# daigo0927/pwcnet

Hardware: AMD Instinct MI355X
Metric: image_pairs_per_sec_448x1024 (higher is better)
Workload: dtype f32 via fp16x2-split MFMA (fp32 tensors and accumulation; big stride-1 convs, level-1 extractor and correlation on the F16 pipe)

## Files before the change

### include/pwc_hip.h

```cpp
#ifndef PWC_HIP_H
#define PWC_HIP_H

#include <stddef.h>
#include <stdint.h>

#ifdef __cplusplus
extern "C" {
#endif

typedef void* pwc_stream_t;

enum {
    PWC_OK = 0,
    PWC_EINVAL = -1,
    PWC_EALIGN = -2,
    PWC_ERANGE = -3,
    PWC_EUNSUPPORTED = -4
};

int pwc_version(void);
const char* pwc_error_string(int code);

int pwc_cost_volume_f32(const float* f0, int f0_cs, const float* f1w, int f1w_cs,
                        float* out, int out_cs, int N, int H, int W, int C,
// ... 86 lines not shown
size_t pwc_conv3x3_h2_workspace_floats(int N, int H, int W, int Cin_phys, int Cout, int dilation);
int pwc_conv3x3_h2_supported(int N, int H, int W, int Cin_phys, int Cout, int dilation);
#define PWC_STATUS_NONFINITE 1u
#define PWC_STATUS_STREAMK_TIMEOUT 2u
int pwc_conv3x3_h2_ex_f32(const float* x, int x_cs, int Cin_a_phys, const float* x2, int x2_cs,
                          const float* packed_w, const float* bias, float* y, int y_cs, int N, int H, int W,
                          int Cin_phys, int Cout, int dilation, int apply_act, float slope, float* workspace,
                          size_t workspace_floats, uint32_t* status, pwc_stream_t stream);
int pwc_conv3x3_h2_ex3_f32(const float* x, int x_cs, int Cin_a_phys, const float* x2, int x2_cs, int Cin_b_phys,
                           const float* x3, int x3_cs, const float* packed_w, const float* bias, float* y, int y_cs,
                           int N, int H, int W, int Cin_phys, int Cout, int apply_act, float slope, float* workspace,
                           size_t workspace_floats, uint32_t* status, pwc_stream_t stream);
size_t pwc_conv3x3_c16pair_packed_floats(void);
int pwc_conv3x3_c16pair_pack_f32(const float* w1_hwio, const float* w2_hwio, float* packed, pwc_stream_t stream);
int pwc_conv3x3_c16pair_f32(const float* x, int x_cs, const float* packed, const float* bias1, const float* bias2,
                            float* y, int y_cs, int N, int H, int W, float slope, pwc_stream_t stream);
int pwc_conv3x3_c16pair_supported(int N, int H, int W);
size_t pwc_conv3x3_c3c16pair_packed_floats(void);
int pwc_conv3x3_c3c16pair_pack_f32(const float* w0_hwio, const float* w1_hwio, const float* w2_hwio, float* packed,
                                   pwc_stream_t stream);
int pwc_conv3x3_c3c16pair_f32(const float* x_a, int N_a, const float* x_b, int N_b, const float* packed,
                              const float* bias0, const float* bias1, const float* bias2, float* y, int y_cs,
                              int H0, int W0, float slope, pwc_stream_t stream);
int pwc_conv3x3_c3c16pair_supported(int N, int H0, int W0);
size_t pwc_conv3x3_h2_stride2_packed_floats(int Cin_phys, int Cout);
int pwc_conv3x3_h2_stride2_pack_f32(const float* w_hwio, const int32_t* cin_map, int Cin, int Cin_phys,
                                    int Cout, float* packed_w, pwc_stream_t stream);
size_t pwc_conv3x3_h2_stride2_workspace_floats(int N, int H, int W, int Cin_phys, int Cout);
int pwc_conv3x3_h2_stride2_f32(const float* x, int x_cs, const float* packed_w, const float* bias,
                               float* y, int y_cs, int N, int H, int W, int Cin_phys, int Cout,
                               int apply_act, float slope, float* workspace, size_t workspace_floats,
                               uint32_t* status, pwc_stream_t stream);
int pwc_conv3x3_h2_stride2_supported(int N, int H, int W, int Cin_phys, int Cout);

size_t pwc_conv3x3_sk_packed_floats(int Cin_phys, int Cout);
int pwc_conv3x3_sk_pack_f32(const float* w_hwio, const int32_t* cin_map, int Cin, int Cin_phys, int Cout,
                            float* packed_w, pwc_stream_t stream);
int pwc_conv3x3_sk_f32(const float* x, int x_cs, const float* packed_w, const float* bias, float* y, int y_cs,
                       int N, int H, int W, int Cin_phys, int Cout, int stride, int dilation, int apply_act,
                       float slope, pwc_stream_t stream);
int pwc_conv3x3_sk_supported(int N, int H, int W, int Cin_phys, int Cout, int stride, int dilation);
int pwc_conv3x3_sk_variant_f32(const float* x, int x_cs, const float* packed_w, const float* bias, float* y, int y_cs,
                               int N, int H, int W, int Cin_phys, int Cout, int stride, int dilation, int apply_act,
                               float slope, int tile, pwc_stream_t stream);

size_t pwc_conv3x3_t32_packed_floats(int Cin_phys);
int pwc_conv3x3_t32_pack_f32(const float* w_hwio, const int32_t* cin_map, int Cin, int Cin_phys, float* packed_w,
                             pwc_stream_t stream);
int pwc_conv3x3_t32_f32(const float* x, int x_cs, const float* packed_w, const float* bias, float* y, int y_cs,
                        int N, int H, int W, int Cin_phys, int Cout, int stride, int apply_act, float slope,
                        pwc_stream_t stream);
int pwc_conv3x3_t32_supported(int N, int H, int W, int Cin_phys, int Cout, int stride);
size_t pwc_conv3x3_w32_packed_floats(int Cin_phys);
int pwc_conv3x3_w32_pack_f32(const float* w_hwio, const int32_t* cin_map, int Cin, int Cin_phys, float* packed_w,
                             pwc_stream_t stream);
int pwc_conv3x3_w32_f32(const float* x, int x_cs, const float* packed_w, const float* bias, float* y, int y_cs,
                        int N, int H, int W, int Cin_phys, int Cout, int apply_act, float slope, pwc_stream_t stream);
int pwc_conv3x3_w32_supported(int N, int H, int W, int Cin_phys, int Cout, int stride, int dilation);
int pwc_conv3x3_h2_plan(int N, int H, int W, int Cin_phys, int Cout, int dilation);
int pwc_conv3x3_h2_variant_f32(const float* x, int x_cs, const float* packed_w, const float* bias,
                               float* y, int y_cs, int N, int H, int W, int Cin_phys, int Cout,
                               int dilation, int apply_act, float slope, int variant, float* workspace,
                               size_t workspace_floats, pwc_stream_t stream);
int pwc_conv3x3_wino_split_plan(int N, int H, int W, int Cin_phys, int Cout, int dilation);
size_t pwc_conv3x3_wino_split_workspace_floats(int N, int H, int W, int Cout, int csplit);
int pwc_conv3x3_wino_split_f32(const float* x, int x_cs, const float* packed_u, const float* bias,
// ... 176 lines not shown
```

### pwcnet_amd/_lib.py

```python
import ctypes
import os
import subprocess

import torch

_HERE = os.path.dirname(os.path.abspath(__file__))
CSRC = os.path.join(_HERE, "csrc")
HARNESS = os.environ.get("PWC_HARNESS", "") == "1"
LIB_PATH = os.path.join(CSRC, "libpwc_hip_harness.so" if HARNESS else "libpwc_hip.so")
HARNESS_SIGNATURES_NAMES = ("pwc_debug_cost_volume_blk_rows", "pwc_debug_conv3x3_sk_tile", "pwc_debug_conv3x3_t32",
                            "pwc_debug_h2_reserve_cus", "pwc_debug_conv3x3_s2_tile")
SOURCES = ["conv3x3_mfma.hip", "conv3x3_wino.hip", "conv3x3_direct.hip", "cost_volume.hip", "pwc_ops.hip",
           "pwc_backward.hip", "conv3x3_wgrad.hip", "conv3x3_h2.hip", "conv3x3_c16pair.hip", "conv3x3_sk.hip", "conv3x3_s2.hip", "conv3x3_t32.hip", "conv3x3_w32.hip",
           "pwc_flow_loss.hip", "pwc_unsup.hip", "pwc_census.hip", "pwc_ssim.hip", "pwc_fbcheck.hip", "pwc_fit.hip", "pwc_augment.hip", "pwc_splat.hip", "pwc_pyramid.hip"]
HEADERS = ["pwc_common.h", "conv_fp32_common.h", "cost_volume_common.h", "loss_common.h", "cost_volume_roll.hip", "cost_volume_mfma.hip", "cost_volume_h2.hip", "cost_volume_blk.hip", "conv3x3_wino4.hip", os.path.join("..", "..", "include", "pwc_hip.h")]

_vp, _i, _f, _l, _sz = ctypes.c_void_p, ctypes.c_int, ctypes.c_float, ctypes.c_long, ctypes.c_size_t

SIGNATURES = {
    "pwc_version": (_i, []),
    "pwc_error_string": (ctypes.c_char_p, [_i]),
    "pwc_cost_volume_f32": (_i, [_vp, _i, _vp, _i, _vp, _i, _i, _i, _i, _i, _i, _f, _vp]),
    "pwc_cost_volume_uses_rolling_kernel": (_i, [_i, _i, _i, _i, _i, _i, _i]),
    "pwc_warp_bilinear_f32": (_i, [_vp, _i, _vp, _i, _f, _vp, _i, _i, _i, _i, _i, _vp]),
    "pwc_warp_nearest_f32": (_i, [_vp, _i, _vp, _i, _f, _vp, _i, _i, _i, _i, _i, _vp]),
    "pwc_cost_volume_coarse_f32": (_i, [_vp, _i, _vp, _i, _vp, _i, _f, _vp, _i, _vp, _i, _i, _i, _i, _i, _i, _f, _vp]),
    "pwc_resize_bilinear_pair_f32": (_i, [_vp, _i, _vp, _i, _vp, _i, _vp, _i, _i, _i, _i, _i, _i, _i, _vp]),
    "pwc_warp_copy_f32": (_i, [_i, _vp, _i, _vp, _i, _f, _vp, _i, _i, _i, _i, _i, _vp, _i, _vp, _i, _i, _vp]),
    "pwc_warp_cost_volume_f32": (_i, [_vp, _i, _vp, _i, _vp, _i, _f, _vp, _i, _i, _i, _i, _i, _i, _f, _vp]),
    "pwc_warp_cost_volume_concat_f32": (_i, [_vp, _i, _vp, _i, _vp, _i, _f, _vp, _i, _i, _vp, _i, _i, _i, _i, _i, _i, _f, _vp]),
    "pwc_warp_cost_volume_concat_h2_f32": (_i, [_vp, _i, _vp, _i, _vp, _i, _f, _vp, _i, _i, _vp, _i, _i, _i, _i, _i, _i, _f, _vp]),
    "pwc_warp_cost_volume_concat_blk_f32": (_i, [_vp, _i, _vp, _i, _vp, _i, _f, _vp, _i, _i, _vp, _i, _i, _i, _i, _i, _i, _f, _vp]),
    "pwc_warp_cost_volume_concat_supported": (_i, [_i, _i, _i, _i, _i, _i, _i, _i, _i]),
    "pwc_warp_cost_volume_concat_blk_supported": (_i, [_i, _i, _i, _i, _i, _i, _i, _i, _i]),
    "pwc_conv3x3_packed_floats": (_sz, [_i, _i]),
    "pwc_conv3x3_pack_f32": (_i, [_vp, _vp, _i, _i, _i, _vp, _vp]),
    "pwc_conv3x3_f32": (_i, [_vp, _i, _vp, _vp, _vp, _i, _i, _i, _i, _i, _i, _i, _i, _i, _f, _i, _i, _vp, _sz, _vp]),
    "pwc_conv3x3_workspace_floats": (_sz, [_i, _i]),
    "pwc_conv3x3_plan": (_i, [_i, _i, _i, ctypes.POINTER(_i)]),
    "pwc_conv3x3_uses_halo_kernel": (_i, [_i, _i, _i, _i, _i]),
    "pwc_conv3x3_tile_shape": (_i, [_i, ctypes.POINTER(_i), ctypes.POINTER(_i)]),
    "pwc_conv3x3_wino_packed_floats": (_sz, [_i, _i]),
    "pwc_conv3x3_wino_pack_f32": (_i, [_vp, _vp, _i, _i, _i, _vp, _vp]),
    "pwc_conv3x3_wino_f32": (_i, [_vp, _i, _vp, _vp, _vp, _i, _i, _i, _i, _i, _i, _i, _i, _f, _vp]),
    "pwc_conv3x3_wino_workgroups": (_l, [_i, _i, _i, _i, _i]),
    "pwc_conv3x3_wino4_packed_floats": (_sz, [_i, _i]),
    "pwc_conv3x3_wino4_pack_f32": (_i, [_vp, _vp, _i, _i, _i, _vp, _vp]),
    "pwc_conv3x3_wino4_f32": (_i, [_vp, _i, _vp, _vp, _vp, _i, _i, _i, _i, _i, _i, _i, _i, _f, _vp]),
    "pwc_conv3x3_wino4_supported": (_i, [_i, _i, _i, _i, _i, _i]),
    "pwc_conv3x3_h2_packed_floats": (_sz, [_i, _i]),
    "pwc_conv3x3_h2_pack_f32": (_i, [_vp, _vp, _i, _i, _i, _vp, _vp]),
    "pwc_conv3x3_h2_f32": (_i, [_vp, _i, _vp, _vp, _vp, _i, _i, _i, _i, _i, _i, _i, _i, _f, _vp, _sz, _vp]),
    "pwc_conv3x3_h2_ex_f32": (_i, [_vp, _i, _i, _vp, _i, _vp, _vp, _vp, _i, _i, _i, _i, _i, _i, _i, _i, _f, _vp, _sz, _vp, _vp]),
    "pwc_conv3x3_h2_ex3_f32": (_i, [_vp, _i, _i, _vp, _i, _i, _vp, _i, _vp, _vp, _vp, _i, _i, _i, _i, _i, _i, _i, _f, _vp, _sz, _vp, _vp]),
    "pwc_conv3x3_h2_workspace_floats": (_sz, [_i, _i, _i, _i, _i, _i]),
    "pwc_conv3x3_h2_supported": (_i, [_i, _i, _i, _i, _i, _i]),
    "pwc_conv3x3_h2_plan": (_i, [_i, _i, _i, _i, _i, _i]),
    "pwc_conv3x3_h2_stride2_f32": (_i, [_vp, _i, _vp, _vp, _vp, _i, _i, _i, _i, _i, _i, _i, _f, _vp, _sz, _vp, _vp]),
    "pwc_conv3x3_h2_stride2_supported": (_i, [_i, _i, _i, _i, _i]),
    "pwc_conv3x3_sk_packed_floats": (_sz, [_i, _i]),
    "pwc_conv3x3_sk_pack_f32": (_i, [_vp, _vp, _i, _i, _i, _vp, _vp]),
    "pwc_conv3x3_sk_f32": (_i, [_vp, _i, _vp, _vp, _vp, _i, _i, _i, _i, _i, _i, _i, _i, _i, _f, _vp]),
    "pwc_conv3x3_sk_supported": (_i, [_i, _i, _i, _i, _i, _i, _i]),
    "pwc_conv3x3_sk_variant_f32": (_i, [_vp, _i, _vp, _vp, _vp, _i, _i, _i, _i, _i, _i, _i, _i, _i, _f, _i, _vp]),
    "pwc_conv3x3_t32_packed_floats": (_sz, [_i]),
    "pwc_conv3x3_t32_pack_f32": (_i, [_vp, _vp, _i, _i, _vp, _vp]),
    "pwc_conv3x3_t32_f32": (_i, [_vp, _i, _vp, _vp, _vp, _i, _i, _i, _i, _i, _i, _i, _i, _f, _vp]),
    "pwc_conv3x3_t32_supported": (_i, [_i, _i, _i, _i, _i, _i]),
    "pwc_conv3x3_w32_packed_floats": (_sz, [_i]),
    "pwc_conv3x3_w32_pack_f32": (_i, [_vp, _vp, _i, _i, _vp, _vp]),
    "pwc_conv3x3_w32_f32": (_i, [_vp, _i, _vp, _vp, _vp, _i, _i, _i, _i, _i, _i, _i, _f, _vp]),
    "pwc_conv3x3_w32_supported": (_i, [_i, _i, _i, _i, _i, _i, _i]),
    "pwc_conv3x3_h2_stride2_packed_floats": (_sz, [_i, _i]),
    "pwc_conv3x3_h2_stride2_pack_f32": (_i, [_vp, _vp, _i, _i, _i, _vp, _vp]),
    "pwc_conv3x3_h2_stride2_workspace_floats": (_sz, [_i, _i, _i, _i, _i]),
    "pwc_conv3x3_c16pair_packed_floats": (_sz, []),
    "pwc_conv3x3_c16pair_pack_f32": (_i, [_vp, _vp, _vp, _vp]),
    "pwc_conv3x3_c16pair_f32": (_i, [_vp, _i, _vp, _vp, _vp, _vp, _i, _i, _i, _i, _f, _vp]),
    "pwc_conv3x3_c16pair_supported": (_i, [_i, _i, _i]),
    "pwc_conv3x3_c3c16pair_packed_floats": (_sz, []),
    "pwc_conv3x3_c3c16pair_pack_f32": (_i, [_vp, _vp, _vp, _vp, _vp]),
    "pwc_conv3x3_c3c16pair_f32": (_i, [_vp, _i, _vp, _i, _vp, _vp, _vp, _vp, _vp, _i, _i, _i, _f, _vp]),
    "pwc_conv3x3_c3c16pair_supported": (_i, [_i, _i, _i]),
    "pwc_conv3x3_h2_variant_f32": (_i, [_vp, _i, _vp, _vp, _vp, _i, _i, _i, _i, _i, _i, _i, _i, _f, _i, _vp, _sz, _vp]),
    "pwc_conv3x3_wino_split_plan": (_i, [_i, _i, _i, _i, _i, _i]),
    "pwc_conv3x3_wino_split_workspace_floats": (_sz, [_i, _i, _i, _i, _i]),
    "pwc_conv3x3_wino_split_f32": (_i, [_vp, _i, _vp, _vp, _vp, _i, _i, _i, _i, _i, _i, _i, _i, _f, _i, _vp, _sz, _vp]),
    "pwc_conv3x3_direct_f32": (_i, [_vp, _i, _vp, _vp, _vp, _i, _vp, _i, _i, _i, _i, _i, _i, _i, _i, _i, _f, _vp]),
    "pwc_resize_bilinear_f32": (_i, [_vp, _i, _vp, _i, _i, _i, _i, _i, _i, _i, _f, _vp]),
    "pwc_resize_bilinear_status_f32": (_i, [_vp, _i, _vp, _i, _i, _i, _i, _i, _i, _i, _f, _vp, _vp]),
    "pwc_absmax_f32": (_i, [_vp, _i, _l, _i, _vp, _vp]),
    "pwc_copy_channels_f32": (_i, [_vp, _i, _vp, _i, _l, _i, _vp]),
# ... 140 lines not shown
```

### pwcnet_amd/csrc/conv3x3_h2.hip

```cpp
#pragma once
#include "pwc_common.h"
#include <type_traits>

typedef float pwc_f32x16 __attribute__((ext_vector_type(16)));

struct H2Args {
    const float* x;
    const void* wp;
    const float* bias;
    float* y;
    int x_cs, y_cs;
    int N, H, W;
    int Cin_phys, Cout;
    int apply_act;
    float slope;
    int tiles_x, tiles_y, ncb;
    int dil_y, dil_x;
    int ntiles;
    float* ws_partial;
    unsigned* dbg;
    int Ho, Wo;
    const float* x2;
    int x2_cs, nc16_a;
    const float* x3;
// ... 590 lines not shown
static unsigned* h2_debug_counters = nullptr;
#else
constexpr unsigned* h2_debug_counters = nullptr;
#endif

template <int CT, int PT, int WCG, int ABL, int XS = 1, bool S2 = false>
static int h2_launch(H2Args& a, int hs, int ws, float* workspace, size_t workspace_floats, hipStream_t stream) {
    typedef H2Cfg<CT, PT, WCG, XS> C;
    a.tiles_x = (ws + 31) / 32; a.tiles_y = (hs + C::TR - 1) / C::TR; a.ncb = a.Cout / (32 * C::NCT);
    const long nblk = (long)a.N * a.dil_y * a.dil_x * a.tiles_x * a.tiles_y * a.ncb;
    if (nblk * (a.Cin_phys >> 4) >= (1L << 31)) return PWC_ERANGE;
    a.ntiles = (int)nblk;
    const int cus = h2_cu_count();
    int grid = a.ntiles;
    a.ws_partial = nullptr;
    const size_t part = (size_t)C::NCT * 32 * C::TR * 32;
    if (workspace && h2_split_pays(a.ntiles, a.Cin_phys >> 4, cus) && workspace_floats >= (size_t)cus * part) {
        grid = cus;
        a.ws_partial = workspace;
    }
    pwc_allow_dynamic_lds<&conv3x3_h2_kernel<CT, PT, WCG, ABL, XS, S2>>(C::LDS);
    hipLaunchKernelGGL((conv3x3_h2_kernel<CT, PT, WCG, ABL, XS, S2>), dim3((unsigned)grid), dim3(512), C::LDS, stream, a);
    return pwc_launch_status();
}

static bool h2s2_tile_routed(int N, int H, int W, int x_cs, int Cin_phys, int Cout) {
    const bool ok = h2s2_has_tile_image(Cin_phys, Cout) && pwc_conv3x3_s2_tile_admits(N, H, W, x_cs, Cin_phys, Cout);
#ifdef PWC_HARNESS
    if (pwc_conv3x3_s2_tile_debug_mode()) return ok && pwc_conv3x3_s2_tile_debug_mode() > 0;
#endif
    return ok && Cin_phys == 32;
}

template <int ABL = 0>
static int h2_run(const float* x, int x_cs, const float* packed_w, const float* bias, float* y, int y_cs, int N, int H, int W,
                  int Cin_phys, int Cout, int dilation, int apply_act, float slope, pwc_stream_t stream, int variant = 0,
                  float* workspace = nullptr, size_t workspace_floats = 0, int stride = 1, const float* x2 = nullptr, int x2_cs = 0,
                  int Cin_a_phys = 0, uint32_t* status = nullptr, const float* x3 = nullptr, int x3_cs = 0, int Cin_b_phys = 0) {
    if (!x || !packed_w || !bias || !y) return PWC_EINVAL;
    if (x3 && !x2) return PWC_EINVAL;
    const int slack = x3 ? 12 : 0;
    if (x2) {
        const int cb = x3 ? Cin_b_phys : Cin_phys - Cin_a_phys;
        if (Cin_a_phys <= 0 || Cin_a_phys >= Cin_phys || (Cin_a_phys % 16) || x_cs < Cin_a_phys - slack || x2_cs < cb - slack) return PWC_EINVAL;
        if ((x2_cs & 3) || !pwc_aligned16(x2)) return PWC_EALIGN;
        if ((long)H * W * x2_cs * 4 >= (long)PWC_OOB) return PWC_ERANGE;
    }
    if (x3) {
        const int cc = Cin_phys - Cin_a_phys - Cin_b_phys;
        if (Cin_b_phys <= 0 || (Cin_b_phys % 16) || cc <= 0 || x3_cs < cc - 12 || dilation != 1) return PWC_EINVAL;
        if ((x3_cs & 3) || !pwc_aligned16(x3)) return PWC_EALIGN;
        if ((long)H * W * x3_cs * 4 >= (long)PWC_OOB) return PWC_ERANGE;
    }
    if (reinterpret_cast<uintptr_t>(status) & 7u) return PWC_EALIGN;
    if (dilation < 1 || (stride != 1 && stride != 2)) return PWC_EINVAL;
    const bool shape_ok = !(Cin_phys % 16 || Cout % 32 || Cout > H2_MAX_COUT || (stride == 2 && (dilation != 1 || (H & 1) || (W & 1) || x2)));
    if (const int rc = pwc_conv_io_check(x, x_cs, x2 ? Cin_a_phys - slack : Cin_phys, y, y_cs, Cout, packed_w, bias, N, H, W, shape_ok)) return rc;
    if (!pwc_aligned16(workspace)) return PWC_EALIGN;
    if (((long)H * W + W + 2) * x_cs * 4 >= (long)PWC_OOB || (long)H * W * y_cs * 4 >= (long)PWC_OOB) return PWC_ERANGE;
    H2Args a;
    a.x = x; a.wp = packed_w; a.bias = bias; a.y = y; a.x_cs = x_cs; a.y_cs = y_cs;
    a.N = N; a.H = H; a.W = W; a.Cin_phys = Cin_phys; a.Cout = Cout; a.apply_act = apply_act; a.slope = slope;
    const bool s2 = stride == 2;
    a.Ho = s2 ? H / 2 : H; a.Wo = s2 ? W / 2 : W;
    if (s2) a.Cin_phys = 4 * Cin_phys;
    const H2Geo geo = h2_geometry(a.Ho, a.Wo, dilation, Cout);
    a.dil_y = geo.dy; a.dil_x = geo.dx;
    a.dbg = h2_debug_counters;
    a.x2 = x2; a.x2_cs = x2_cs; a.nc16_a = x2 ? Cin_a_phys >> 4 : a.Cin_phys >> 4; a.status = status;
    a.x3 = x3; a.x3_cs = x3_cs; a.nc16_b = x3 ? Cin_b_phys >> 4 : (a.Cin_phys >> 4) - a.nc16_a;
    const int hs = geo.hs, ws = geo.ws;
    if (variant == 0) variant = h2_plan(N, a.Ho, a.Wo, a.Cin_phys, Cout, dilation, nullptr);
    if (variant < 1 || variant > 5) return PWC_EUNSUPPORTED;
    if (Cout % h2_variant(variant).couts) return PWC_EUNSUPPORTED;
    if (s2 && h2s2_tile_routed(N, H, W, x_cs, Cin_phys, Cout))
        return pwc_conv3x3_s2_tile_launch(x, x_cs, packed_w + h2s2_tile_image_offset(Cin_phys, Cout), bias, y, y_cs, N, H, W, Cin_phys,
                                          Cout, apply_act, slope, stream);
    if (s2) {
        switch (variant) {
            case 1: return h2_launch<2, 2, 2, ABL, 1, true>(a, hs, ws, workspace, workspace_floats, (hipStream_t)stream);
            case 2: return h2_launch<2, 2, 1, ABL, 1, true>(a, hs, ws, workspace, workspace_floats, (hipStream_t)stream);
            case 3: return h2_launch<3, 1, 1, ABL, 1, true>(a, hs, ws, workspace, workspace_floats, (hipStream_t)stream);
            case 4: return h2_launch<1, 2, 1, ABL, 1, true>(a, hs, ws, workspace, workspace_floats, (hipStream_t)stream);
            default: return h2_launch<1, 2, 2, ABL, 1, true>(a, hs, ws, workspace, workspace_floats, (hipStream_t)stream);
        }
    }
    if (geo.xs == 2) {
        switch (variant) {
            case 1: return h2_launch<2, 2, 2, ABL, 2>(a, hs, ws, workspace, workspace_floats, (hipStream_t)stream);
            case 3: return h2_launch<3, 1, 1, ABL, 2>(a, hs, ws, workspace, workspace_floats, (hipStream_t)stream);
            case 5: return h2_launch<1, 2, 2, ABL, 2>(a, hs, ws, workspace, workspace_floats, (hipStream_t)stream);
            default: return PWC_EUNSUPPORTED;
        }
    }
    switch (variant) {
        case 1: return h2_launch<2, 2, 2, ABL>(a, hs, ws, workspace, workspace_floats, (hipStream_t)stream);
        case 2: return h2_launch<2, 2, 1, ABL>(a, hs, ws, workspace, workspace_floats, (hipStream_t)stream);
        case 3: return h2_launch<3, 1, 1, ABL>(a, hs, ws, workspace, workspace_floats, (hipStream_t)stream);
        case 4: return h2_launch<1, 2, 1, ABL>(a, hs, ws, workspace, workspace_floats, (hipStream_t)stream);
        default: return h2_launch<1, 2, 2, ABL>(a, hs, ws, workspace, workspace_floats, (hipStream_t)stream);
    }
}

extern "C" size_t pwc_conv3x3_h2_workspace_floats(int N, int H, int W, int Cin_phys, int Cout, int dilation) {
// ... 62 lines not shown
```

### pwcnet_amd/csrc/conv3x3_s2.hip

```cpp
#include "pwc_common.h"

typedef unsigned int s2_u32x4 __attribute__((ext_vector_type(4)));
#define S2_OOB 0x80000000u

constexpr int S2_PC = 2 * PWC_S2_TILE_COLS + 1;
constexpr int S2_PR = 2 * PWC_S2_TILE_ROWS + 1;
constexpr int S2_NPX = S2_PR * S2_PC;
constexpr int S2_EVEN = PWC_S2_TILE_COLS + 1;
constexpr int S2_LINE = S2_PC * 32;
constexpr int S2_CC = 64;
constexpr int S2_UB = 5;

struct S2Args {
    const float* x;
    const float* wp;
    const float* bias;
    float* y;
    int x_cs, y_cs;
    int N, H, W, Ho, Wo;
    int Cin_phys, Cout;
    int pad_t, pad_l;
    int apply_act;
    float slope;
    int ntx, nty;
    int cg;
    int nsteps;
};

template <int NBW>
__global__ __launch_bounds__(512) void conv3x3_s2_kernel(const S2Args a) {
    extern __shared__ __attribute__((aligned(16))) char s2_smem[];
    const int t = threadIdx.x, lane = t & 63;
    const int wave = __builtin_amdgcn_readfirstlane(t >> 6);
    int b = blockIdx.x;
    const int tx = b % a.ntx;
    b /= a.ntx;
    const int ty = b % a.nty, n = b / a.nty;

    const __amdgpu_buffer_rsrc_t rx = __builtin_amdgcn_make_buffer_rsrc(
        (void*)a.x, 0, (int)((size_t)a.N * a.H * a.W * a.x_cs * 4), 0x00020000);
    const __amdgpu_buffer_rsrc_t rw = __builtin_amdgcn_make_buffer_rsrc(
        (void*)a.wp, 0, (int)((size_t)a.Cout * a.nsteps * 128), 0x00020000);
    const int m = lane & 15, kq = lane >> 4;
    const int row = wave >> 1, cb0 = (wave & 1) * NBW, nb = a.Cout >> 4;

    f32x4 hh[2][NBW], xx[2][NBW];
#pragma unroll
    for (int hf = 0; hf < 2; ++hf)
#pragma unroll
        for (int j = 0; j < NBW; ++j) {
            hh[hf][j] = f32x4{0.f, 0.f, 0.f, 0.f};
            xx[hf][j] = f32x4{0.f, 0.f, 0.f, 0.f};
        }

    auto fetch_b = [&](s2_u32x4 (&bv)[NBW][2], int s, bool live) {
#pragma unroll
        for (int j = 0; j < NBW; ++j) {
            const int cb = cb0 + j;
            const unsigned vo = (live && cb < nb) ? (unsigned)((cb * a.nsteps + s) * 2048 + lane * 16) : S2_OOB;
            bv[j][0] = __builtin_amdgcn_raw_buffer_load_b128(rw, (int)vo, 0, 0);
            bv[j][1] = __builtin_amdgcn_raw_buffer_load_b128(rw, (int)vo, 1024, 0);
        }
    };

    const int gy0 = 2 * PWC_S2_TILE_ROWS * ty - a.pad_t, gx0 = 2 * PWC_S2_TILE_COLS * tx - a.pad_l;
    for (int c0 = 0; c0 < a.Cin_phys; c0 += S2_CC) {
        const int cc = a.Cin_phys - c0 < S2_CC ? a.Cin_phys - c0 : S2_CC;
        const int cgc = cc >> 5, ng16 = cc >> 4, cqs = 1 + cgc;
        const int nst = 9 * cgc, sbase = c0 >> 5;
        auto gstep = [&](int si) { const int tap = si / cgc; return tap * a.cg + sbase + (si - tap * cgc); };
        if (c0) __syncthreads();
        s2_u32x4 b0[NBW][2], b1[NBW][2];
        fetch_b(b0, gstep(0), true);
        const int nu = S2_NPX << cqs;
#pragma unroll 1
        for (int u0 = t; u0 < nu; u0 += 512 * S2_UB) {
            f32x4 v[S2_UB][2];
            int dst[S2_UB];
#pragma unroll
            for (int k = 0; k < S2_UB; ++k) {
                const int u = u0 + 512 * k;
                const int px = u >> cqs, j = u - (px << cqs);
                const int pr = px / S2_PC, pc = px - pr * S2_PC;
                const int gy = gy0 + pr, gx = gx0 + pc;
                const bool ok = u < nu && (unsigned)gy < (unsigned)a.H && (unsigned)gx < (unsigned)a.W;
                const unsigned vo = ok ? (unsigned)(((n * a.H + gy) * a.W + gx) * a.x_cs + c0 + j * 8) * 4u : S2_OOB;
                v[k][0] = __builtin_bit_cast(f32x4, __builtin_amdgcn_raw_buffer_load_b128(rx, (int)vo, 0, 0));
                v[k][1] = __builtin_bit_cast(f32x4, __builtin_amdgcn_raw_buffer_load_b128(rx, (int)vo, 16, 0));
                const int pos = (pc & 1) ? S2_EVEN + (pc >> 1) : pc >> 1;
                dst[k] = u < nu ? ((pr * ng16 + (j >> 1)) * 2) * S2_LINE + pos * 32 + (j & 1) * 16 : -1;
            }
#pragma unroll
            for (int k = 0; k < S2_UB; ++k)
                if (dst[k] >= 0) {
                    pwc_f16x4 h0, m0, h1, m1;
                    pwc_split4(v[k][0], h0, m0);
                    pwc_split4(v[k][1], h1, m1);
                    *reinterpret_cast<pwc_f16x8*>(s2_smem + dst[k]) = __builtin_shufflevector(h0, h1, 0, 1, 2, 3, 4, 5, 6, 7);
                    *reinterpret_cast<pwc_f16x8*>(s2_smem + dst[k] + S2_LINE) = __builtin_shufflevector(m0, m1, 0, 1, 2, 3, 4, 5, 6, 7);
                }
        }
        __syncthreads();

        auto step = [&](const s2_u32x4 (&bv)[NBW][2], int si) {
            const int tap = si / cgc, c32 = si - tap * cgc;
            const int dy = tap / 3, dx = tap - 3 * dy;
            const int pos = (dx == 1 ? S2_EVEN : 0) + (dx >> 1) + m;
            const char* p = s2_smem + (((2 * row + dy) * ng16 + 2 * c32 + (kq >> 1)) * 2) * S2_LINE + pos * 32 + (kq & 1) * 16;
            pwc_f16x8 ah[2], am[2];
#pragma unroll
            for (int hf = 0; hf < 2; ++hf) {
                ah[hf] = *reinterpret_cast<const pwc_f16x8*>(p + hf * 512);
                am[hf] = *reinterpret_cast<const pwc_f16x8*>(p + hf * 512 + S2_LINE);
            }
#pragma unroll
            for (int j = 0; j < NBW; ++j) {
                const pwc_f16x8 wh = __builtin_bit_cast(pwc_f16x8, bv[j][0]);
                const pwc_f16x8 wm = __builtin_bit_cast(pwc_f16x8, bv[j][1]);
#pragma unroll
                for (int hf = 0; hf < 2; ++hf) {
                    xx[hf][j] = __builtin_amdgcn_mfma_f32_16x16x32_f16(wm, ah[hf], xx[hf][j], 0, 0, 0);
                    hh[hf][j] = __builtin_amdgcn_mfma_f32_16x16x32_f16(wh, ah[hf], hh[hf][j], 0, 0, 0);
                    xx[hf][j] = __builtin_amdgcn_mfma_f32_16x16x32_f16(wh, am[hf], xx[hf][j], 0, 0, 0);
                }
            }
        };
#pragma unroll 1
        for (int si = 0; si < nst; si += 2) {
            fetch_b(b1, gstep(si + 1 < nst ? si + 1 : 0), si + 1 < nst);
            step(b0, si);
            fetch_b(b0, gstep(si + 2 < nst ? si + 2 : 0), si + 2 < nst);
            if (si + 1 < nst) step(b1, si + 1);
        }
    }

    const int oy = PWC_S2_TILE_ROWS * ty + row;
#pragma unroll
    for (int hf = 0; hf < 2; ++hf) {
        const int ox = PWC_S2_TILE_COLS * tx + hf * 16 + m;
        if (oy < a.Ho && ox < a.Wo) {
            float* yp = a.y + ((size_t)(n * a.Ho + oy) * a.Wo + ox) * a.y_cs + 4 * kq;
#pragma unroll
            for (int j = 0; j < NBW; ++j) {
                const int cb = cb0 + j;
                if (cb < nb) {
                    f32x4 v = __builtin_elementwise_fma(xx[hf][j], f32x4{1.f / 2048.f, 1.f / 2048.f, 1.f / 2048.f, 1.f / 2048.f}, hh[hf][j]);
                    v += *reinterpret_cast<const f32x4*>(a.bias + cb * 16 + 4 * kq);
                    if (a.apply_act) v = pwc_lrelu4(v, a.slope);
                    *reinterpret_cast<f32x4*>(yp + cb * 16) = v;
                }
            }
        }
    }
}

template <int NBW>
static int s2_launch(const S2Args& a, hipStream_t s) {
    const long wgs = (long)a.N * a.nty * a.ntx;
    if (wgs >= (1L << 31)) return PWC_ERANGE;
    const int cc = a.Cin_phys < S2_CC ? a.Cin_phys : S2_CC;
    pwc_allow_dynamic_lds<&conv3x3_s2_kernel<NBW>>(S2_NPX * S2_CC * 4);
    hipLaunchKernelGGL((conv3x3_s2_kernel<NBW>), dim3((unsigned)wgs), dim3(512), (size_t)S2_NPX * cc * 4, s, a);
    return pwc_launch_status();
}

bool pwc_conv3x3_s2_tile_admits(int N, int H, int W, int x_cs, int Cin_phys, int Cout) {
    if (N <= 0 || H <= 0 || W <= 0 || Cin_phys <= 0 || Cout <= 0 || x_cs < Cin_phys) return false;
    if (Cin_phys % 32 || Cout % 16 || Cout > 128) return false;
    return pwc_fits_2g(N, H, W, x_cs) && (long)Cout * 9 * (Cin_phys / 32) * 128 < (1L << 31);
}

long pwc_conv3x3_s2_tile_count(int N, int H, int W) {
    const int Ho = (H + 1) / 2, Wo = (W + 1) / 2;
    return (long)N * ((Ho + PWC_S2_TILE_ROWS - 1) / PWC_S2_TILE_ROWS) * ((Wo + PWC_S2_TILE_COLS - 1) / PWC_S2_TILE_COLS);
}

int pwc_conv3x3_s2_tile_launch(const float* x, int x_cs, const float* packed_w, const float* bias, float* y, int y_cs, int N, int H,
                               int W, int Cin_phys, int Cout, int apply_act, float slope, pwc_stream_t stream) {
    if (!pwc_conv3x3_s2_tile_admits(N, H, W, x_cs, Cin_phys, Cout)) return PWC_EUNSUPPORTED;
    S2Args a;
    a.x = x; a.wp = packed_w; a.bias = bias; a.y = y; a.x_cs = x_cs; a.y_cs = y_cs;
    a.N = N; a.H = H; a.W = W;
    pwc_same_pad(H, 2, 1, &a.Ho, &a.pad_t);
    pwc_same_pad(W, 2, 1, &a.Wo, &a.pad_l);
    a.Cin_phys = Cin_phys; a.Cout = Cout; a.apply_act = apply_act; a.slope = slope;
    a.ntx = (a.Wo + PWC_S2_TILE_COLS - 1) / PWC_S2_TILE_COLS;
    a.nty = (a.Ho + PWC_S2_TILE_ROWS - 1) / PWC_S2_TILE_ROWS;
    a.cg = Cin_phys / 32; a.nsteps = 9 * a.cg;
    hipStream_t s = (hipStream_t)stream;
    switch ((Cout / 16 + 1) / 2) {
        case 1: return s2_launch<1>(a, s);
        case 2: return s2_launch<2>(a, s);
        case 3: return s2_launch<3>(a, s);
        default: return s2_launch<4>(a, s);
    }
}

#ifdef PWC_HARNESS
static int s2_tile_mode = 0;
extern "C" int pwc_debug_conv3x3_s2_tile(int mode) { s2_tile_mode = mode; return 0; }
int pwc_conv3x3_s2_tile_debug_mode() { return s2_tile_mode; }
#endif
```

### pwcnet_amd/csrc/pwc_common.h

```cpp
#pragma once
#include <hip/hip_runtime.h>
#include <stdint.h>

#include "../../include/pwc_hip.h"

typedef float f32x4 __attribute__((ext_vector_type(4)));
typedef float f32x2 __attribute__((ext_vector_type(2)));
typedef _Float16 pwc_f16x8 __attribute__((ext_vector_type(8)));
typedef _Float16 pwc_f16x4 __attribute__((ext_vector_type(4)));
typedef _Float16 pwc_f16x2 __attribute__((ext_vector_type(2)));

#define PWC_WAVE 64

static inline int pwc_launch_status() {
    hipError_t e = hipGetLastError();
    return e == hipSuccess ? PWC_OK : (int)e;
}

template <auto Kernel>
static inline void pwc_allow_dynamic_lds(int bytes) {
    static unsigned long long done[4] = {0, 0, 0, 0};
    int d = 0;
    if (hipGetDevice(&d) == hipSuccess && d >= 0 && d < 256) {
        const unsigned long long bit = 1ull << (d & 63);
// ... 125 lines not shown
__device__ __forceinline__ void pwc_split4(const float x0, const float x1, const float x2, const float x3, pwc_f16x4& h, pwc_f16x4& m) {
    pwc_split4(f32x4{x0, x1, x2, x3}, h, m);
}
__device__ __forceinline__ void pwc_split1(const float x, _Float16& h, _Float16& m) {
    h = (_Float16)x;
    m = (_Float16)__builtin_fmaf((float)h, -2048.f, x * 2048.f);
}

template <int COUT = 32>
__global__ void conv3x3_c32_pack_kernel(const float* __restrict__ w, const int32_t* __restrict__ cin_map, int Cin, int Cin_phys,
                                        _Float16* __restrict__ packed) {
    static_assert(COUT == 32, "the row operand of v_mfma_f32_32x32x16_f16");
    const int j16 = Cin_phys >> 4;
    const int total = 9 * j16 * 512;
    for (int idx = blockIdx.x * blockDim.x + threadIdx.x; idx < total; idx += gridDim.x * blockDim.x) {
        const int e = idx & 7, lane = (idx >> 3) & 63;
        const int r = idx >> 9;
        const int j = r % j16, tap = r / j16;
        const int cphys = j * 16 + (lane >> 5) * 8 + e, co = lane & (COUT - 1);
        const int clog = cin_map ? cin_map[cphys] : (cphys < Cin ? cphys : -1);
        float v = 0.f;
        if (clog >= 0 && clog < Cin) v = w[((size_t)tap * Cin + clog) * COUT + co];
        _Float16* dst = packed + (size_t)r * 1024 + lane * 8 + e;
        pwc_split1(v, dst[0], dst[512]);
    }
}

#define PWC_S2_TILE_ROWS 4
#define PWC_S2_TILE_COLS 32
bool pwc_conv3x3_s2_tile_admits(int N, int H, int W, int x_cs, int Cin_phys, int Cout);
long pwc_conv3x3_s2_tile_count(int N, int H, int W);
int pwc_conv3x3_s2_tile_launch(const float* x, int x_cs, const float* packed_w, const float* bias, float* y, int y_cs, int N, int H,
                               int W, int Cin_phys, int Cout, int apply_act, float slope, pwc_stream_t stream);
#ifdef PWC_HARNESS
int pwc_conv3x3_s2_tile_debug_mode();
#endif
```

Before: 3593.

## Add single-pass stride-1 tiled conv kernel for small 64/96-channel h2 layers

Adds a stride-1 3x3 convolution kernel, modelled on the existing stride-2 tile kernel. Each 512-thread workgroup stages a 6x34 halo tile of the whole 64- or 96-channel input in LDS as fp16 hi/lo splits. It then runs all 9*CG MFMA steps from that tile, with weights prefetched by buffer loads one or two steps ahead. The h2 dispatcher routes dilation-1 64->64 and 96->96 convs to it when the tile count falls in a mid range (under 256 tiles), aiming to raise occupancy and cut per-step overhead on small coarse-pyramid layers. Shared MMA, store and split helpers are factored out of the s2 kernel, and the routing thresholds are heuristic and may misroute some shapes.

```diff
diff --git a/include/pwc_hip.h b/include/pwc_hip.h
--- a/include/pwc_hip.h
+++ b/include/pwc_hip.h
@@ -142,6 +142,10 @@
                                int apply_act, float slope, float* workspace, size_t workspace_floats,
                                uint32_t* status, pwc_stream_t stream);
 int pwc_conv3x3_h2_stride2_supported(int N, int H, int W, int Cin_phys, int Cout);
+int pwc_conv3x3_s1_tile_f32(const float* x, int x_cs, const float* packed_w, const float* bias,
+                            float* y, int y_cs, int N, int H, int W, int Cin_phys, int Cout,
+                            int dilation, int apply_act, float slope, pwc_stream_t stream);
+int pwc_conv3x3_h2_uses_s1_tile(int N, int H, int W, int x_cs, int Cin_phys, int Cout, int dilation);
 
 size_t pwc_conv3x3_sk_packed_floats(int Cin_phys, int Cout);
 int pwc_conv3x3_sk_pack_f32(const float* w_hwio, const int32_t* cin_map, int Cin, int Cin_phys, int Cout,
diff --git a/pwcnet_amd/_lib.py b/pwcnet_amd/_lib.py
--- a/pwcnet_amd/_lib.py
+++ b/pwcnet_amd/_lib.py
@@ -9,7 +9,7 @@
 HARNESS = os.environ.get("PWC_HARNESS", "") == "1"
 LIB_PATH = os.path.join(CSRC, "libpwc_hip_harness.so" if HARNESS else "libpwc_hip.so")
 HARNESS_SIGNATURES_NAMES = ("pwc_debug_cost_volume_blk_rows", "pwc_debug_conv3x3_sk_tile", "pwc_debug_conv3x3_t32",
-                            "pwc_debug_h2_reserve_cus", "pwc_debug_conv3x3_s2_tile")
+                            "pwc_debug_h2_reserve_cus", "pwc_debug_conv3x3_s2_tile", "pwc_debug_conv3x3_s1_tile")
 SOURCES = ["conv3x3_mfma.hip", "conv3x3_wino.hip", "conv3x3_direct.hip", "cost_volume.hip", "pwc_ops.hip",
            "pwc_backward.hip", "conv3x3_wgrad.hip", "conv3x3_h2.hip", "conv3x3_c16pair.hip", "conv3x3_sk.hip", "conv3x3_s2.hip", "conv3x3_t32.hip", "conv3x3_w32.hip",
            "pwc_flow_loss.hip", "pwc_unsup.hip", "pwc_census.hip", "pwc_ssim.hip", "pwc_fbcheck.hip", "pwc_fit.hip", "pwc_augment.hip", "pwc_splat.hip", "pwc_pyramid.hip"]
@@ -58,6 +58,8 @@
     "pwc_conv3x3_h2_plan": (_i, [_i, _i, _i, _i, _i, _i]),
     "pwc_conv3x3_h2_stride2_f32": (_i, [_vp, _i, _vp, _vp, _vp, _i, _i, _i, _i, _i, _i, _i, _f, _vp, _sz, _vp, _vp]),
     "pwc_conv3x3_h2_stride2_supported": (_i, [_i, _i, _i, _i, _i]),
+    "pwc_conv3x3_s1_tile_f32": (_i, [_vp, _i, _vp, _vp, _vp, _i, _i, _i, _i, _i, _i, _i, _i, _f, _vp]),
+    "pwc_conv3x3_h2_uses_s1_tile": (_i, [_i, _i, _i, _i, _i, _i, _i]),
     "pwc_conv3x3_sk_packed_floats": (_sz, [_i, _i]),
     "pwc_conv3x3_sk_pack_f32": (_i, [_vp, _vp, _i, _i, _i, _vp, _vp]),
     "pwc_conv3x3_sk_f32": (_i, [_vp, _i, _vp, _vp, _vp, _i, _i, _i, _i, _i, _i, _i, _i, _i, _f, _vp]),
diff --git a/pwcnet_amd/csrc/conv3x3_h2.hip b/pwcnet_amd/csrc/conv3x3_h2.hip
--- a/pwcnet_amd/csrc/conv3x3_h2.hip
+++ b/pwcnet_amd/csrc/conv3x3_h2.hip
@@ -646,6 +646,25 @@
     return ok && Cin_phys == 32;
 }
 
+#define PWC_H2_S1_TILE_MAX 256L
+#define PWC_H2_S1_TILE_MIN_64_64 56L
+#define PWC_H2_S1_TILE_MIN_96_96 28L
+static bool h2_s1_tile_routed(int N, int H, int W, int x_cs, int Cin_phys, int Cout, int dilation) {
+    const bool ok = dilation == 1 && pwc_conv3x3_s1_tile_admits(N, H, W, x_cs, Cin_phys, Cout);
+#ifdef PWC_HARNESS
+    if (pwc_conv3x3_s1_tile_debug_mode()) return ok && pwc_conv3x3_s1_tile_debug_mode() > 0;
+#endif
+    if (!ok) return false;
+    const long tiles = pwc_conv3x3_s1_tile_count(N, H, W);
+    if (tiles > PWC_H2_S1_TILE_MAX) return false;
+    if (Cin_phys == 64 && Cout == 64) return tiles >= PWC_H2_S1_TILE_MIN_64_64;
+    if (Cin_phys == 96 && Cout == 96) return tiles >= PWC_H2_S1_TILE_MIN_96_96;
+    return false;
+}
+extern "C" int pwc_conv3x3_h2_uses_s1_tile(int N, int H, int W, int x_cs, int Cin_phys, int Cout, int dilation) {
+    return h2_s1_tile_routed(N, H, W, x_cs, Cin_phys, Cout, dilation) ? 1 : 0;
+}
+
 template <int ABL = 0>
 static int h2_run(const float* x, int x_cs, const float* packed_w, const float* bias, float* y, int y_cs, int N, int H, int W,
                   int Cin_phys, int Cout, int dilation, int apply_act, float slope, pwc_stream_t stream, int variant = 0,
@@ -684,6 +703,8 @@
     a.x2 = x2; a.x2_cs = x2_cs; a.nc16_a = x2 ? Cin_a_phys >> 4 : a.Cin_phys >> 4; a.status = status;
     a.x3 = x3; a.x3_cs = x3_cs; a.nc16_b = x3 ? Cin_b_phys >> 4 : (a.Cin_phys >> 4) - a.nc16_a;
     const int hs = geo.hs, ws = geo.ws;
+    if (ABL == 0 && variant == 0 && !s2 && !x2 && h2_s1_tile_routed(N, H, W, x_cs, Cin_phys, Cout, dilation))
+        return pwc_conv3x3_s1_tile_launch(x, x_cs, packed_w, bias, y, y_cs, N, H, W, Cin_phys, Cout, apply_act, slope, stream);
     if (variant == 0) variant = h2_plan(N, a.Ho, a.Wo, a.Cin_phys, Cout, dilation, nullptr);
     if (variant < 1 || variant > 5) return PWC_EUNSUPPORTED;
     if (Cout % h2_variant(variant).couts) return PWC_EUNSUPPORTED;
diff --git a/pwcnet_amd/csrc/conv3x3_s2.hip b/pwcnet_amd/csrc/conv3x3_s2.hip
--- a/pwcnet_amd/csrc/conv3x3_s2.hip
+++ b/pwcnet_amd/csrc/conv3x3_s2.hip
@@ -27,6 +27,50 @@
     int nsteps;
 };
 
+__device__ __forceinline__ void s2_put_unit(char* dst, int line, const f32x4 v0, const f32x4 v1) {
+    pwc_f16x4 h0, m0, h1, m1;
+    pwc_split4(v0, h0, m0);
+    pwc_split4(v1, h1, m1);
+    *reinterpret_cast<pwc_f16x8*>(dst) = __builtin_shufflevector(h0, h1, 0, 1, 2, 3, 4, 5, 6, 7);
+    *reinterpret_cast<pwc_f16x8*>(dst + line) = __builtin_shufflevector(m0, m1, 0, 1, 2, 3, 4, 5, 6, 7);
+}
+template <int NBW>
+__device__ __forceinline__ void s2_mma(const s2_u32x4 (&bv)[NBW][2], const pwc_f16x8 (&ah)[2], const pwc_f16x8 (&am)[2],
+                                       f32x4 (&hh)[2][NBW], f32x4 (&xx)[2][NBW]) {
+#pragma unroll
+    for (int j = 0; j < NBW; ++j) {
+        const pwc_f16x8 wh = __builtin_bit_cast(pwc_f16x8, bv[j][0]);
+        const pwc_f16x8 wm = __builtin_bit_cast(pwc_f16x8, bv[j][1]);
+#pragma unroll
+        for (int hf = 0; hf < 2; ++hf) {
+            xx[hf][j] = __builtin_amdgcn_mfma_f32_16x16x32_f16(wm, ah[hf], xx[hf][j], 0, 0, 0);
+            hh[hf][j] = __builtin_amdgcn_mfma_f32_16x16x32_f16(wh, ah[hf], hh[hf][j], 0, 0, 0);
+            xx[hf][j] = __builtin_amdgcn_mfma_f32_16x16x32_f16(wh, am[hf], xx[hf][j], 0, 0, 0);
+        }
+    }
+}
+template <int NBW>
+__device__ __forceinline__ void s2_store(const S2Args& a, int n, int oy, int ox0, int m, int kq, int cb0, int nb,
+                                         const f32x4 (&hh)[2][NBW], const f32x4 (&xx)[2][NBW]) {
+#pragma unroll
+    for (int hf = 0; hf < 2; ++hf) {
+        const int ox = ox0 + hf * 16 + m;
+        if (oy < a.Ho && ox < a.Wo) {
+            float* yp = a.y + ((size_t)(n * a.Ho + oy) * a.Wo + ox) * a.y_cs + 4 * kq;
+#pragma unroll
+            for (int j = 0; j < NBW; ++j) {
+                const int cb = cb0 + j;
+                if (cb < nb) {
+                    f32x4 v = __builtin_elementwise_fma(xx[hf][j], f32x4{1.f / 2048.f, 1.f / 2048.f, 1.f / 2048.f, 1.f / 2048.f}, hh[hf][j]);
+                    v += *reinterpret_cast<const f32x4*>(a.bias + cb * 16 + 4 * kq);
+                    if (a.apply_act) v = pwc_lrelu4(v, a.slope);
+                    *reinterpret_cast<f32x4*>(yp + cb * 16) = v;
+                }
+            }
+        }
+    }
+}
+
 template <int NBW>
 __global__ __launch_bounds__(512) void conv3x3_s2_kernel(const S2Args a) {
     extern __shared__ __attribute__((aligned(16))) char s2_smem[];
@@ -92,13 +136,7 @@
             }
 #pragma unroll
             for (int k = 0; k < S2_UB; ++k)
-                if (dst[k] >= 0) {
-                    pwc_f16x4 h0, m0, h1, m1;
-                    pwc_split4(v[k][0], h0, m0);
-                    pwc_split4(v[k][1], h1, m1);
-                    *reinterpret_cast<pwc_f16x8*>(s2_smem + dst[k]) = __builtin_shufflevector(h0, h1, 0, 1, 2, 3, 4, 5, 6, 7);
-                    *reinterpret_cast<pwc_f16x8*>(s2_smem + dst[k] + S2_LINE) = __builtin_shufflevector(m0, m1, 0, 1, 2, 3, 4, 5, 6, 7);
-                }
+                if (dst[k] >= 0) s2_put_unit(s2_smem + dst[k], S2_LINE, v[k][0], v[k][1]);
         }
         __syncthreads();
 
@@ -113,17 +151,7 @@
                 ah[hf] = *reinterpret_cast<const pwc_f16x8*>(p + hf * 512);
                 am[hf] = *reinterpret_cast<const pwc_f16x8*>(p + hf * 512 + S2_LINE);
             }
-#pragma unroll
-            for (int j = 0; j < NBW; ++j) {
-                const pwc_f16x8 wh = __builtin_bit_cast(pwc_f16x8, bv[j][0]);
-                const pwc_f16x8 wm = __builtin_bit_cast(pwc_f16x8, bv[j][1]);
-#pragma unroll
-                for (int hf = 0; hf < 2; ++hf) {
-                    xx[hf][j] = __builtin_amdgcn_mfma_f32_16x16x32_f16(wm, ah[hf], xx[hf][j], 0, 0, 0);
-                    hh[hf][j] = __builtin_amdgcn_mfma_f32_16x16x32_f16(wh, ah[hf], hh[hf][j], 0, 0, 0);
-                    xx[hf][j] = __builtin_amdgcn_mfma_f32_16x16x32_f16(wh, am[hf], xx[hf][j], 0, 0, 0);
-                }
-            }
+            s2_mma<NBW>(bv, ah, am, hh, xx);
         };
 #pragma unroll 1
         for (int si = 0; si < nst; si += 2) {
@@ -134,24 +162,7 @@
         }
     }
 
-    const int oy = PWC_S2_TILE_ROWS * ty + row;
-#pragma unroll
-    for (int hf = 0; hf < 2; ++hf) {
-        const int ox = PWC_S2_TILE_COLS * tx + hf * 16 + m;
-        if (oy < a.Ho && ox < a.Wo) {
-            float* yp = a.y + ((size_t)(n * a.Ho + oy) * a.Wo + ox) * a.y_cs + 4 * kq;
-#pragma unroll
-            for (int j = 0; j < NBW; ++j) {
-                const int cb = cb0 + j;
-                if (cb < nb) {
-                    f32x4 v = __builtin_elementwise_fma(xx[hf][j], f32x4{1.f / 2048.f, 1.f / 2048.f, 1.f / 2048.f, 1.f / 2048.f}, hh[hf][j]);
-                    v += *reinterpret_cast<const f32x4*>(a.bias + cb * 16 + 4 * kq);
-                    if (a.apply_act) v = pwc_lrelu4(v, a.slope);
-                    *reinterpret_cast<f32x4*>(yp + cb * 16) = v;
-                }
-            }
-        }
-    }
+    s2_store<NBW>(a, n, PWC_S2_TILE_ROWS * ty + row, PWC_S2_TILE_COLS * tx, m, kq, cb0, nb, hh, xx);
 }
 
 template <int NBW>
@@ -196,8 +207,163 @@
     }
 }
 
+constexpr int S1_PC = PWC_S1_TILE_COLS + 2;
+constexpr int S1_PR = PWC_S1_TILE_ROWS + 2;
+constexpr int S1_NPX = S1_PR * S1_PC;
+constexpr int S1_LINE = (S1_PC + 1) * 32;
+
+template <int NBW, int CG>
+__global__ __launch_bounds__(512, NBW <= 2 ? 4 : 2) void conv3x3_s1_kernel(const S2Args a) {
+    extern __shared__ __attribute__((aligned(16))) char s1_smem[];
+    constexpr int NG16 = 2 * CG, NST = 9 * CG, NPU = 4 * CG;
+    constexpr int NU = S1_NPX * NPU, UB = (NU + 511) / 512;
+    constexpr int AHEAD = NBW <= 2 ? 1 : 2;
+    const int t = threadIdx.x, lane = t & 63;
+    const int wave = __builtin_amdgcn_readfirstlane(t >> 6);
+    int b = blockIdx.x;
+    const int tx = b % a.ntx;
+    b /= a.ntx;
+    const int ty = b % a.nty, n = b / a.nty;
+
+    const int nct = a.Cout >> 5;
+    const __amdgpu_buffer_rsrc_t rx = __builtin_amdgcn_make_buffer_rsrc(
+        (void*)a.x, 0, (int)((size_t)a.N * a.H * a.W * a.x_cs * 4), 0x00020000);
+    const __amdgpu_buffer_rsrc_t rw = __builtin_amdgcn_make_buffer_rsrc(
+        (void*)a.wp, 0, NG16 * nct * 9 * 2048, 0x00020000);
+    const int m = lane & 15, kq = lane >> 4;
+    const int row = wave >> 1, cb0 = (wave & 1) * NBW, nb = a.Cout >> 4;
+
+    f32x4 hh[2][NBW], xx[2][NBW];
+#pragma unroll
+    for (int hf = 0; hf < 2; ++hf)
+#pragma unroll
+        for (int j = 0; j < NBW; ++j) {
+            hh[hf][j] = f32x4{0.f, 0.f, 0.f, 0.f};
+            xx[hf][j] = f32x4{0.f, 0.f, 0.f, 0.f};
+        }
+
+    const unsigned wlane = (unsigned)((kq >> 1) * (nct * 9 * 2048) + (kq & 1) * 512 + m * 16);
+    auto fetch_b = [&](s2_u32x4 (&bv)[NBW][2], int s) {
+        const int tap = s / CG, c32 = s - tap * CG;
+        const int dy = tap / 3, dx = tap - 3 * dy;
+#pragma unroll
+        for (int j = 0; j < NBW; ++j) {
+            const int cb = cb0 + j;
+            const unsigned vo = cb < nb ? (unsigned)((((6 * c32 + dy) * nct + (cb >> 1)) * 3 + dx) * 2048 + (cb & 1) * 256) + wlane : S2_OOB;
+            bv[j][0] = __builtin_amdgcn_raw_buffer_load_b128(rw, (int)vo, 0, 0);
+            bv[j][1] = __builtin_amdgcn_raw_buffer_load_b128(rw, (int)vo, 1024, 0);
+        }
+    };
+    s2_u32x4 bw[AHEAD + 1][NBW][2];
+#pragma unroll
+    for (int s = 0; s < AHEAD; ++s) fetch_b(bw[s], s);
+
+    {
+        const int gy0 = PWC_S1_TILE_ROWS * ty - 1, gx0 = PWC_S1_TILE_COLS * tx - 1;
+        f32x4 v[UB][2];
+        int dst[UB];
+#pragma unroll
+        for (int k = 0; k < UB; ++k) {
+            const int u = t + 512 * k;
+            const int px = u / NPU, j = u - px * NPU;
+            const int pr = px / S1_PC, pc = px - pr * S1_PC;
+            const int gy = gy0 + pr, gx = gx0 + pc;
+            const bool ok = u < NU && (unsigned)gy < (unsigned)a.H && (unsigned)gx < (unsigned)a.W;
+            const unsigned vo = ok ? (unsigned)(((n * a.H + gy) * a.W + gx) * a.x_cs + j * 8) * 4u : S2_OOB;
+            v[k][0] = __builtin_bit_cast(f32x4, __builtin_amdgcn_raw_buffer_load_b128(rx, (int)vo, 0, 0));
+            v[k][1] = __builtin_bit_cast(f32x4, __builtin_amdgcn_raw_buffer_load_b128(rx, (int)vo, 16, 0));
+            dst[k] = u < NU ? ((pr * NG16 + (j >> 1)) * 2) * S1_LINE + pc * 32 + (j & 1) * 16 : -1;
+        }
+#pragma unroll
+        for (int k = 0; k < UB; ++k)
+            if (dst[k] >= 0) s2_put_unit(s1_smem + dst[k], S1_LINE, v[k][0], v[k][1]);
+    }
+    __syncthreads();
+
+    const char* const pl = s1_smem + ((row * NG16 + (kq >> 1)) * 2) * S1_LINE + m * 32 + (kq & 1) * 16;
+#pragma unroll
+    for (int si = 0; si < NST; ++si) {
+        if (si + AHEAD < NST) fetch_b(bw[(si + AHEAD) % (AHEAD + 1)], si + AHEAD);
+        const int tap = si / CG, c32 = si - tap * CG;
+        const int dy = tap / 3, dx = tap - 3 * dy;
+        const char* p = pl + ((dy * NG16 + 2 * c32) * 2) * S1_LINE + dx * 32;
+        pwc_f16x8 ah[2], am[2];
+#pragma unroll
+        for (int hf = 0; hf < 2; ++hf) {
+            ah[hf] = *reinterpret_cast<const pwc_f16x8*>(p + hf * 512);
+            am[hf] = *reinterpret_cast<const pwc_f16x8*>(p + hf * 512 + S1_LINE);
+        }
+        s2_mma<NBW>(bw[si % (AHEAD + 1)], ah, am, hh, xx);
+    }
+    s2_store<NBW>(a, n, PWC_S1_TILE_ROWS * ty + row, PWC_S1_TILE_COLS * tx, m, kq, cb0, nb, hh, xx);
+}
+
+template <int NBW, int CG>
+static int s1_launch(const S2Args& a, hipStream_t s) {
+    const long wgs = (long)a.N * a.nty * a.ntx;
+    if (wgs >= (1L << 31)) return PWC_ERANGE;
+    constexpr int lds = S1_PR * 2 * CG * 2 * S1_LINE;
+    pwc_allow_dynamic_lds<&conv3x3_s1_kernel<NBW, CG>>(lds);
+    hipLaunchKernelGGL((conv3x3_s1_kernel<NBW, CG>), dim3((unsigned)wgs), dim3(512), (size_t)lds, s, a);
+    return pwc_launch_status();
+}
+
+bool pwc_conv3x3_s1_tile_shape_ok(int Cin_phys, int Cout) {
+    return (Cin_phys == 64 || Cin_phys == 96) && Cout >= 32 && Cout <= 128 && Cout % 32 == 0;
+}
+
+bool pwc_conv3x3_s1_tile_admits(int N, int H, int W, int x_cs, int Cin_phys, int Cout) {
+    if (N <= 0 || H <= 0 || W <= 0 || x_cs < Cin_phys || !pwc_conv3x3_s1_tile_shape_ok(Cin_phys, Cout)) return false;
+    return pwc_fits_2g(N, H, W, x_cs);
+}
+
+long pwc_conv3x3_s1_tile_count(int N, int H, int W) {
+    return (long)N * ((H + PWC_S1_TILE_ROWS - 1) / PWC_S1_TILE_ROWS) * ((W + PWC_S1_TILE_COLS - 1) / PWC_S1_TILE_COLS);
+}
+
+int pwc_conv3x3_s1_tile_launch(const float* x, int x_cs, const float* packed_w, const float* bias, float* y, int y_cs, int N, int H,
+                               int W, int Cin_phys, int Cout, int apply_act, float slope, pwc_stream_t stream) {
+    if (!pwc_conv3x3_s1_tile_admits(N, H, W, x_cs, Cin_phys, Cout)) return PWC_EUNSUPPORTED;
+    S2Args a;
+    a.x = x; a.wp = packed_w; a.bias = bias; a.y = y; a.x_cs = x_cs; a.y_cs = y_cs;
+    a.N = N; a.H = H; a.W = W; a.Ho = H; a.Wo = W; a.pad_t = 1; a.pad_l = 1;
+    a.Cin_phys = Cin_phys; a.Cout = Cout; a.apply_act = apply_act; a.slope = slope;
+    a.ntx = (W + PWC_S1_TILE_COLS - 1) / PWC_S1_TILE_COLS;
+    a.nty = (H + PWC_S1_TILE_ROWS - 1) / PWC_S1_TILE_ROWS;
+    a.cg = Cin_phys / 32; a.nsteps = 9 * a.cg;
+    hipStream_t s = (hipStream_t)stream;
+    const int nbw = Cout / 32;
+    if (Cin_phys == 64) {
+        switch (nbw) {
+            case 1: return s1_launch<1, 2>(a, s);
+            case 2: return s1_launch<2, 2>(a, s);
+            case 3: return s1_launch<3, 2>(a, s);
+            default: return s1_launch<4, 2>(a, s);
+        }
+    }
+    switch (nbw) {
+        case 1: return s1_launch<1, 3>(a, s);
+        case 2: return s1_launch<2, 3>(a, s);
+        case 3: return s1_launch<3, 3>(a, s);
+        default: return s1_launch<4, 3>(a, s);
+    }
+}
+
+extern "C" int pwc_conv3x3_s1_tile_f32(const float* x, int x_cs, const float* packed_w, const float* bias, float* y, int y_cs, int N,
+                                       int H, int W, int Cin_phys, int Cout, int dilation, int apply_act, float slope,
+                                       pwc_stream_t stream) {
+    if (dilation < 1) return PWC_EINVAL;
+    const bool shape_ok = dilation == 1 && pwc_conv3x3_s1_tile_shape_ok(Cin_phys, Cout);
+    if (const int rc = pwc_conv_io_check(x, x_cs, Cin_phys, y, y_cs, Cout, packed_w, bias, N, H, W, shape_ok)) return rc;
+    if (!pwc_fits_2g(N, H, W, x_cs)) return PWC_ERANGE;
+    return pwc_conv3x3_s1_tile_launch(x, x_cs, packed_w, bias, y, y_cs, N, H, W, Cin_phys, Cout, apply_act, slope, stream);
+}
+
 #ifdef PWC_HARNESS
 static int s2_tile_mode = 0;
 extern "C" int pwc_debug_conv3x3_s2_tile(int mode) { s2_tile_mode = mode; return 0; }
 int pwc_conv3x3_s2_tile_debug_mode() { return s2_tile_mode; }
+static int s1_tile_mode = 0;
+extern "C" int pwc_debug_conv3x3_s1_tile(int mode) { s1_tile_mode = mode; return 0; }
+int pwc_conv3x3_s1_tile_debug_mode() { return s1_tile_mode; }
 #endif
diff --git a/pwcnet_amd/csrc/pwc_common.h b/pwcnet_amd/csrc/pwc_common.h
--- a/pwcnet_amd/csrc/pwc_common.h
+++ b/pwcnet_amd/csrc/pwc_common.h
@@ -181,6 +181,14 @@
 long pwc_conv3x3_s2_tile_count(int N, int H, int W);
 int pwc_conv3x3_s2_tile_launch(const float* x, int x_cs, const float* packed_w, const float* bias, float* y, int y_cs, int N, int H,
                                int W, int Cin_phys, int Cout, int apply_act, float slope, pwc_stream_t stream);
+#define PWC_S1_TILE_ROWS 4
+#define PWC_S1_TILE_COLS 32
+bool pwc_conv3x3_s1_tile_shape_ok(int Cin_phys, int Cout);
+bool pwc_conv3x3_s1_tile_admits(int N, int H, int W, int x_cs, int Cin_phys, int Cout);
+long pwc_conv3x3_s1_tile_count(int N, int H, int W);
+int pwc_conv3x3_s1_tile_launch(const float* x, int x_cs, const float* packed_w, const float* bias, float* y, int y_cs, int N, int H,
+                               int W, int Cin_phys, int Cout, int apply_act, float slope, pwc_stream_t stream);
 #ifdef PWC_HARNESS
 int pwc_conv3x3_s2_tile_debug_mode();
+int pwc_conv3x3_s1_tile_debug_mode();
 #endif
```

Result: no change. 3600 (median of 5 runs) (+0.2%).
